# jluuser/PyTorch-VAE

Hardware: AMD Instinct MI355X
Metric: train images/sec @64x64x3 bs256 (curve tensors [B,64,6], SURVEY.md s0) (higher is better)
Workload: dtype f32; 1 GPU; C2: stage2_vq.yaml model with num_quantizers=1 K=512 D=64 N=64; full train step (fwd+loss+bwd+clip+AdamW+EMA), dropout 0.1, loss weights at epoch 100; per_gpu_batch=256, global_batch=256, seq_len=64, parallelism=dp1, hipgraph=True, params=43115078

## Files before the change

pytorch-vae_amd/csrc/gemm_dma.inc:

```

namespace dma {
constexpr int TBM = 256, TBN = 128, TBK = 32;
constexpr int A_BYTES = TBM * TBK * 4, B_BYTES = TBN * TBK * 4, STAGE_BYTES = A_BYTES + B_BYTES;
constexpr int NSTAGE = 3, LDS_BYTES = NSTAGE * STAGE_BYTES;
constexpr int DMA_A = A_BYTES / 1024 / 4, DMA_B = B_BYTES / 1024 / 4, DMA_PER_WAVE = DMA_A + DMA_B;
constexpr int MI = 4, NJ = 2;
}

typedef float f32x2 __attribute__((ext_vector_type(2)));

typedef unsigned u32x2 __attribute__((ext_vector_type(2)));
typedef unsigned u32x4 __attribute__((ext_vector_type(4)));
typedef short s16x4 __attribute__((ext_vector_type(4)));
typedef __bf16 bf16x8 __attribute__((ext_vector_type(8)));

namespace x3 {
constexpr int A_PLANE = dma::TBM * dma::TBK * 2, B_PLANE = dma::TBN * dma::TBK * 2;
constexpr int B_OFF = 3 * A_PLANE;
constexpr int STAGE_BYTES = 3 * (A_PLANE + B_PLANE);
constexpr int LDS_BYTES = 2 * STAGE_BYTES;
constexpr int NU = 12, NUA = 8;
constexpr int NB = 8, G = 48, NSLOT = 96;
constexpr int BAR = 7 * NU;
constexpr int RS_OFF = 40960;
static_assert(LDS_BYTES <= dma::LDS_BYTES, "x3 stages must fit the launch's dynamic LDS");
}

template <class F, int... I>
__device__ __forceinline__ void static_for_impl(F&& f, std::integer_sequence<int, I...>) { (f(std::integral_constant<int, I>{}), ...); }
template <int N, class F>
__device__ __forceinline__ void static_for(F&& f) { static_for_impl(f, std::make_integer_sequence<int, N>{}); }

struct SplitUnit {
    float r0, r1, r2, r3;
    unsigned t0, t1, t2, t3;
    unsigned hp[2], mp[2], lp[2];
    template <int S> __device__ __forceinline__ void step(const f32x4& a) {
        if constexpr (S == 0) {
            asm volatile("v_cvt_pk_bf16_f32 %0, %6, %7\n\tv_cvt_pk_bf16_f32 %1, %8, %9\n\tv_lshlrev_b32 %2, 16, %0\n\t"
                         "v_and_b32 %3, 0xffff0000, %0\n\tv_sub_f32 %4, %6, %2\n\tv_sub_f32 %5, %7, %3"
                         : "=&v"(hp[0]), "=&v"(hp[1]), "=&v"(t0), "=&v"(t1), "=&v"(r0), "=&v"(r1)
                         : "v"(a[0]), "v"(a[1]), "v"(a[2]), "v"(a[3]) : "memory");
        } else if constexpr (S == 1) {
            asm volatile("v_lshlrev_b32 %0, 16, %6\n\tv_and_b32 %1, 0xffff0000, %6\n\tv_sub_f32 %2, %7, %0\n\t"
                         "v_sub_f32 %3, %8, %1\n\tv_cvt_pk_bf16_f32 %4, %9, %10\n\tv_cvt_pk_bf16_f32 %5, %2, %3"
                         : "=&v"(t2), "=&v"(t3), "=&v"(r2), "=&v"(r3), "=&v"(mp[0]), "=&v"(mp[1])
                         : "v"(hp[1]), "v"(a[2]), "v"(a[3]), "v"(r0), "v"(r1) : "memory");
        } else if constexpr (S == 2) {
            asm volatile("v_lshlrev_b32 %0, 16, %2\n\tv_and_b32 %1, 0xffff0000, %2" : "=&v"(t0), "=&v"(t1) : "v"(mp[0]) : "memory");
        } else if constexpr (S == 3) {
            asm volatile("v_sub_f32 %0, %0, %2\n\tv_sub_f32 %1, %1, %3" : "+v"(r0), "+v"(r1) : "v"(t0), "v"(t1) : "memory");
        } else if constexpr (S == 4) {
            asm volatile("v_lshlrev_b32 %0, 16, %6\n\tv_and_b32 %1, 0xffff0000, %6\n\tv_sub_f32 %2, %2, %0\n\t"
                         "v_sub_f32 %3, %3, %1\n\tv_cvt_pk_bf16_f32 %4, %7, %8\n\tv_cvt_pk_bf16_f32 %5, %2, %3"
                         : "=&v"(t2), "=&v"(t3), "+v"(r2), "+v"(r3), "=&v"(lp[0]), "=&v"(lp[1])
                         : "v"(mp[1]), "v"(r0), "v"(r1) : "memory");
        }
    }
    __device__ __forceinline__ void all(const f32x4& a) { step<0>(a); step<1>(a); step<2>(a); step<3>(a); step<4>(a); }
};

__device__ __forceinline__ void glds16_s(const char* ubase, unsigned voff, unsigned lds_byte_addr_uniform) {
    asm volatile("s_mov_b32 m0, %2\n\ts_nop 0\n\tglobal_load_lds_dwordx4 %0, %1"
                 :
                 : "v"(voff), "s"(ubase), "s"(lds_byte_addr_uniform)
                 : "memory");
}

__device__ __forceinline__ void glds16(const float* gptr, unsigned lds_byte_addr_uniform) {
    __builtin_amdgcn_global_load_lds(gptr, (__attribute__((address_space(3))) void*)(uintptr_t)lds_byte_addr_uniform, 16, 0, 0);
}

template <bool A_KC, bool B_KC, int MODE, bool X3 = false>
__device__ __forceinline__ void gemm_dma_tile(const GemmArgs& g, const int tile, const int zsplit) {
    using namespace dma;
    constexpr bool EA_KC = X3 ? true : A_KC, EB_KC = X3 ? true : B_KC;
    extern __shared__ __attribute__((aligned(1024))) unsigned char smem_dma[];
    const int tid = threadIdx.x, lane = tid & 63;
    const int wave = __builtin_amdgcn_readfirstlane(tid >> 6);
    const int wm = wave >> 1, wn = wave & 1;
    const int l31 = lane & 31, h = lane >> 5;

    const int tiles_n = g.N / TBN;
    const int m0 = (tile / tiles_n) * TBM, n0 = (tile % tiles_n) * TBN;
    const int kbeg = zsplit * g.kchunk;
    const int kend = min(g.K, kbeg + g.kchunk);
    const int nk = (kend - kbeg) / TBK;

    unsigned voff[DMA_PER_WAVE];
    unsigned dst[DMA_PER_WAVE];
#pragma unroll
    for (int i = 0; i < DMA_A; ++i) {
        const int j = wave + 4 * i;
        if (A_KC) {
            const int R = j * 8 + (lane >> 3), c = (lane & 7) ^ ((R >> 1) & 7);
            voff[i] = (unsigned)(((size_t)R * g.lda + c * 4) * 4);
        } else {
            voff[i] = (unsigned)(((size_t)j * g.lda + lane * 4) * 4);
        }
        dst[i] = j * 1024;
    }
#pragma unroll
    for (int i = 0; i < DMA_B; ++i) {
        const int j = wave + 4 * i;
        if (B_KC) {
            const int R = j * 8 + (lane >> 3), c = (lane & 7) ^ ((R >> 1) & 7);
            voff[DMA_A + i] = (unsigned)(((size_t)R * g.ldb + c * 4) * 4);
        } else {
            voff[DMA_A + i] = (unsigned)(((size_t)(2 * j + (lane >> 5)) * g.ldb + (lane & 31) * 4) * 4);
        }
        dst[DMA_A + i] = A_BYTES + j * 1024;
    }
    const char* baseA = reinterpret_cast<const char*>(A_KC ? g.A + (size_t)m0 * g.lda + kbeg : g.A + (size_t)kbeg * g.lda + m0);
    const char* baseB = reinterpret_cast<const char*>(B_KC ? g.B + (size_t)n0 * g.ldb + kbeg : g.B + (size_t)kbeg * g.ldb + n0);
    const size_t stepA = (A_KC ? (size_t)TBK : (size_t)TBK * g.lda) * 4;
    const size_t stepB = (B_KC ? (size_t)TBK : (size_t)TBK * g.ldb) * 4;
    const unsigned lds0 = (unsigned)(uintptr_t)smem_dma;

    const int sw = (l31 >> 1) & 7;
    unsigned offA[4], offB[4];
#pragma unroll
    for (int t = 0; t < 4; ++t) {
        offA[t] = A_KC ? (unsigned)((wm * 128 + l31) * 128 + (((2 * t + h) ^ sw) * 16))
                       : (unsigned)((8 * t + 4 * h) * (TBM * 4) + (wm * 128 + 4 * l31) * 4);
        offB[t] = A_BYTES + (B_KC ? (unsigned)((wn * 64 + l31) * 128 + (((2 * t + h) ^ sw) * 16))
                                  : (unsigned)((8 * t + 4 * h) * (TBN * 4) + (wn * 64 + 2 * l31) * 4));
    }

    f32x16 acc[MI][NJ];
#pragma unroll
    for (int i = 0; i < MI; ++i)
#pragma unroll
        for (int j = 0; j < NJ; ++j)
#pragma unroll
            for (int r = 0; r < 16; ++r) acc[i][j][r] = 0.f;

    f32x4 fa[2][4];
    f32x4 fbk[2][2];
    f32x2 fbr[2][4];
    const bool do_rowsum = (!A_KC) && (g.rowsum != nullptr) && (n0 == 0) && (X3 || wn == 0);
    float rs[4] = {0.f, 0.f, 0.f, 0.f};

    constexpr int NREAD = 4 + (B_KC ? 2 : 4);
    constexpr int NMF = 4 * MI * NJ;
    constexpr int GAP = NMF / (NREAD + 1);
    auto substep = [&](auto c_c, auto rt_c, auto v0_c, auto v1_c, int rstage, int kt_d, int dstage) {
        constexpr int c = decltype(c_c)::value, RT = decltype(rt_c)::value, V0 = decltype(v0_c)::value,
                      V1 = decltype(v1_c)::value, n = c ^ 1;
        const unsigned char* sb = smem_dma + rstage * STAGE_BYTES;
        const unsigned dsb = lds0 + dstage * STAGE_BYTES;
        if (do_rowsum) {
#pragma unroll
            for (int e = 0; e < 4; ++e)
#pragma unroll
                for (int i = 0; i < 4; ++i) rs[i] += fa[c][e][i];
        }
#pragma unroll
        for (int m = 0; m < NMF; ++m) {
            const int e = m / (MI * NJ), i = (m / NJ) % MI, j = m % NJ;
            const float av = A_KC ? fa[c][i][e] : fa[c][e][i];
            const float bv = B_KC ? fbk[c][j][e] : fbr[c][e][j];
            acc[i][j] = __builtin_amdgcn_mfma_f32_32x32x2f32(av, bv, acc[i][j], 0, 0, 0);
            if ((m % GAP) == 0 && m / GAP < NREAD) {
                const int d = m / GAP;
                if (d < 4) {
                    fa[n][d] = *reinterpret_cast<const f32x4*>(sb + offA[RT] + (A_KC ? d * 32 * 128 : d * TBM * 4));
                } else if (B_KC) {
                    fbk[n][d - 4] = *reinterpret_cast<const f32x4*>(sb + offB[RT] + (d - 4) * 32 * 128);
                } else {
                    fbr[n][d - 4] = *reinterpret_cast<const f32x2*>(sb + offB[RT] + (d - 4) * TBN * 4);
                }
            }
            if ((m % GAP) == GAP / 2 && V0 + m / GAP < V1) {
                const int v = V0 + m / GAP;
                const char* ub = (v < DMA_A) ? baseA + (size_t)kt_d * stepA : baseB + (size_t)kt_d * stepB;
                glds16_s(ub, voff[v], __builtin_amdgcn_readfirstlane(dsb + dst[v]));
            }
        }
#pragma unroll
        for (int m = 0; m < NMF; ++m) {
            __builtin_amdgcn_sched_group_barrier(0x008, 1, 0);
            if ((m % GAP) == 0 && m / GAP < NREAD) __builtin_amdgcn_sched_group_barrier(0x100, 1, 0);
            if ((m % GAP) == GAP / 2 && V0 + m / GAP < V1) __builtin_amdgcn_sched_group_barrier(0x020, 1, 0);
        }
    };
    auto read_first = [&](int rstage) {
        const unsigned char* sb = smem_dma + rstage * STAGE_BYTES;
#pragma unroll
        for (int d = 0; d < 4; ++d) fa[0][d] = *reinterpret_cast<const f32x4*>(sb + offA[0] + (A_KC ? d * 32 * 128 : d * TBM * 4));
        if (B_KC) {
#pragma unroll
            for (int d = 0; d < 2; ++d) fbk[0][d] = *reinterpret_cast<const f32x4*>(sb + offB[0] + d * 32 * 128);
        } else {
#pragma unroll
            for (int d = 0; d < 4; ++d) fbr[0][d] = *reinterpret_cast<const f32x2*>(sb + offB[0] + d * TBN * 4);
        }
    };
    auto issue_all = [&](int kt, int stage) {
        const unsigned sbb = lds0 + stage * STAGE_BYTES;
#pragma unroll
        for (int v = 0; v < DMA_PER_WAVE; ++v) {
            const char* ub = (v < DMA_A) ? baseA + (size_t)kt * stepA : baseB + (size_t)kt * stepB;
            glds16_s(ub, voff[v], __builtin_amdgcn_readfirstlane(sbb + dst[v]));
        }
    };

    const int c4 = (lane & 15) * 4;
    const int col = n0 + wn * 64 + c4;
    constexpr bool HAS_DROP = (MODE == EPI_RELU_DROP || MODE == EPI_DROP_RESID);
    constexpr bool HAS_AUX = (MODE == EPI_DROP_RESID || MODE > EPI_SIGMOID);
    unsigned dkey = 0;
    if (g.drop.p > 0.f && g.drop.rng_state) dkey = drop_key(g.drop, g.drop.rng_state[0], g.drop.rng_state[1]);
    unsigned dmask[4] = {0u, 0u, 0u, 0u};
    const unsigned pair0 = (unsigned)((((unsigned long long)(m0 + wm * 128 + (lane >> 4)) * g.N + col) >> 2) * 2);
    const unsigned g0 = pair0 * 0x9E3779B9U;
    const unsigned gstep = (unsigned)(2 * g.N) * 0x9E3779B9U;
    auto hash_quad = [&](int qi) {
        const unsigned gq = g0 + (unsigned)qi * gstep;
        const unsigned b0 = mix32(dkey ^ gq), b1 = mix32(dkey ^ (gq + 0x9E3779B9U));
        unsigned f4 = ((b0 & 0xffffu) >= g.drop.thr) ? 1u : 0u;
        f4 |= ((b0 >> 16) >= g.drop.thr) ? 2u : 0u;
        f4 |= ((b1 & 0xffffu) >= g.drop.thr) ? 4u : 0u;
        f4 |= ((b1 >> 16) >= g.drop.thr) ? 8u : 0u;
        const unsigned sh = f4 << ((qi & 7) * 4);
        const int w = qi >> 3;
#pragma unroll
        for (int k = 0; k < 4; ++k) dmask[k] |= (w == k) ? sh : 0u;
    };
    f32x4 auxr[32];
    auto load_aux_all = [&]() {
        const float* ap = g.aux_in + (size_t)(m0 + wm * 128 + (lane >> 4)) * g.ldaux + col;
#pragma unroll
        for (int q = 0; q < 32; ++q) auxr[q] = *reinterpret_cast<const f32x4*>(ap + (size_t)(q * 4) * g.ldaux);
    };

    using I0 = std::integral_constant<int, 0>;
    using I1 = std::integral_constant<int, 1>;
    using I2 = std::integral_constant<int, 2>;
    using I3 = std::integral_constant<int, 3>;
    using IH = std::integral_constant<int, DMA_PER_WAVE / 2>;
    using IF = std::integral_constant<int, DMA_PER_WAVE>;
    if constexpr (X3) {
        const unsigned vA = A_KC ? (unsigned)(((size_t)(8 * wave + (lane >> 3)) * g.lda + 4 * (lane & 7)) * 4)
                                 : (unsigned)(((size_t)(8 * wave) * g.lda + 4 * lane) * 4);
        const unsigned vB = B_KC ? (unsigned)(((size_t)(8 * wave + (lane >> 3)) * g.ldb + 4 * (lane & 7)) * 4)
                                 : (unsigned)(((size_t)(8 * wave + (lane >> 5)) * g.ldb + 4 * (lane & 31)) * 4);
        const size_t uA = (A_KC ? (size_t)32 * g.lda : (size_t)g.lda) * 4;
        const size_t uB = (B_KC ? (size_t)32 * g.ldb : (size_t)2 * g.ldb) * 4;
        unsigned wA[4], wB[2];
        {
            const int R = 8 * wave + (lane >> 3), c = (lane & 7) >> 1;
            const unsigned wkc = (unsigned)(R * 64 + ((c ^ ((R >> 2) & 3)) * 16) + (lane & 1) * 8);
#pragma unroll
            for (int x = 0; x < 4; ++x) wA[x] = A_KC ? wkc : (unsigned)((8 * wave) * 512 + (((lane >> 3) ^ x) * 64) + (lane & 7) * 8);
#pragma unroll
            for (int x = 0; x < 2; ++x)
                wB[x] = B_KC ? wkc
                             : (unsigned)((8 * wave + (lane >> 5)) * 256 + ((((lane >> 3) & 3) ^ ((2 * x + (lane >> 5)) & 3)) * 64) + (lane & 7) * 8);
        }
        unsigned rA[4], rB[2];
        {
            const int q = (lane & 15) >> 2, p = lane & 3, sub = (lane >> 4) & 1;
            if (A_KC) {
                const int R = wm * 128 + l31, f = (l31 >> 2) & 3;
                rA[0] = (unsigned)(R * 64 + ((h ^ f) * 16));
                rA[1] = (unsigned)(R * 64 + (((2 + h) ^ f) * 16));
                rA[2] = rA[3] = 0;
            } else {
#pragma unroll
                for (int i = 0; i < 4; ++i) rA[i] = (unsigned)((8 * h + q) * 512 + (((wm * 4 + i) ^ q) * 64) + (16 * sub + 4 * p) * 2);
            }
            if (B_KC) {
                const int R = wn * 64 + l31, f = (l31 >> 2) & 3;
                rB[0] = (unsigned)(R * 64 + ((h ^ f) * 16));
                rB[1] = (unsigned)(R * 64 + (((2 + h) ^ f) * 16));
            } else {
#pragma unroll
                for (int j = 0; j < 2; ++j) rB[j] = (unsigned)((8 * h + q) * 256 + (((wn * 2 + j) ^ q) * 64) + (16 * sub + 4 * p) * 2);
            }
        }
        f32x4 st[x3::NU];
        u32x4 xA[3][4];
        u32x4 xB[2][3][2];
        SplitUnit su;
        auto load_unit = [&](auto u_c, int kt) {
            constexpr int u = decltype(u_c)::value;
            if constexpr (u < x3::NUA) st[u] = *reinterpret_cast<const f32x4*>(baseA + (size_t)kt * stepA + (size_t)u * uA + vA);
            else st[u] = *reinterpret_cast<const f32x4*>(baseB + (size_t)kt * stepB + (size_t)(u - x3::NUA) * uB + vB);
        };
        auto write_unit = [&](auto u_c, auto pl_c, unsigned char* sb) {
            constexpr int u = decltype(u_c)::value, pl = decltype(pl_c)::value;
            const u32x2 v = pl == 0 ? u32x2{su.hp[0], su.hp[1]} : pl == 1 ? u32x2{su.mp[0], su.mp[1]} : u32x2{su.lp[0], su.lp[1]};
            if constexpr (u < x3::NUA) {
                constexpr int cst = A_KC ? u * 2048 : u * 512;
                *reinterpret_cast<u32x2*>(sb + pl * x3::A_PLANE + cst + wA[A_KC ? 0 : (u & 3)]) = v;
            } else {
                constexpr int i = u - x3::NUA;
                constexpr int cst = B_KC ? i * 2048 : 2 * i * 256;
                *reinterpret_cast<u32x2*>(sb + x3::B_OFF + pl * x3::B_PLANE + cst + wB[B_KC ? 0 : (i & 1)]) = v;
            }
        };
        auto read_A = [&](auto pl_c, auto i_c, auto g_c, const unsigned char* sb) -> u32x4 {
            constexpr int pl = decltype(pl_c)::value, i = decltype(i_c)::value, gg = decltype(g_c)::value;
            if constexpr (A_KC) {
                return *reinterpret_cast<const u32x4*>(sb + pl * x3::A_PLANE + i * 2048 + rA[gg]);
            } else {
                const unsigned a0 = (unsigned)(uintptr_t)(sb + pl * x3::A_PLANE + (16 * gg) * 512 + rA[i]);
                const s16x4 lo = __builtin_amdgcn_ds_read_tr16_b64_v4i16((__attribute__((address_space(3))) s16x4*)(uintptr_t)a0);
                const s16x4 hi = __builtin_amdgcn_ds_read_tr16_b64_v4i16((__attribute__((address_space(3))) s16x4*)(uintptr_t)(a0 + 4 * 512));
                const u32x2 l2 = __builtin_bit_cast(u32x2, lo), h2 = __builtin_bit_cast(u32x2, hi);
                return u32x4{l2[0], l2[1], h2[0], h2[1]};
            }
        };
        auto read_B = [&](auto pl_c, auto j_c, auto g_c, const unsigned char* sb) -> u32x4 {
            constexpr int pl = decltype(pl_c)::value, j = decltype(j_c)::value, gg = decltype(g_c)::value;
            if constexpr (B_KC) {
                return *reinterpret_cast<const u32x4*>(sb + x3::B_OFF + pl * x3::B_PLANE + j * 2048 + rB[gg]);
            } else {
                const unsigned a0 = (unsigned)(uintptr_t)(sb + x3::B_OFF + pl * x3::B_PLANE + (16 * gg) * 256 + rB[j]);
                const s16x4 lo = __builtin_amdgcn_ds_read_tr16_b64_v4i16((__attribute__((address_space(3))) s16x4*)(uintptr_t)a0);
                const s16x4 hi = __builtin_amdgcn_ds_read_tr16_b64_v4i16((__attribute__((address_space(3))) s16x4*)(uintptr_t)(a0 + 4 * 256));
                const u32x2 l2 = __builtin_bit_cast(u32x2, lo), h2 = __builtin_bit_cast(u32x2, hi);
                return u32x4{l2[0], l2[1], h2[0], h2[1]};
            }
        };
        auto aux_one = [&](auto q_c) {
            constexpr int q = decltype(q_c)::value;
            auxr[q] = *reinterpret_cast<const f32x4*>(g.aux_in + (size_t)(m0 + wm * 128 + (lane >> 4) + q * 4) * g.ldaux + col);
        };
        if (nk > 0) {
            static_for<x3::NU>([&](auto u_c) { load_unit(u_c, 0); });
            if (HAS_DROP && g.drop.p > 0.f && !g.ws) {
#pragma unroll
                for (int qi = 0; qi < 32; ++qi) hash_quad(qi);
            }
            static_for<x3::NU>([&](auto u_c) {
                constexpr int u = decltype(u_c)::value;
                if (do_rowsum && u < x3::NUA) {
#pragma unroll
                    for (int e = 0; e < 4; ++e) rs[e] += st[u][e];
                }
                su.all(st[u]);
                write_unit(u_c, I0{}, smem_dma);
                write_unit(u_c, I1{}, smem_dma);
                write_unit(u_c, I2{}, smem_dma);
                load_unit(u_c, nk > 1 ? 1 : 0);
            });
            asm volatile("s_waitcnt lgkmcnt(0)" ::: "memory");
            __builtin_amdgcn_s_barrier();
            static_for<4>([&](auto i_c) { xA[0][decltype(i_c)::value] = read_A(I0{}, i_c, I0{}, smem_dma); });
            static_for<6>([&](auto x_c) {
                constexpr int x = decltype(x_c)::value;
                xB[0][x / 2][x % 2] = read_B(std::integral_constant<int, x / 2>{}, std::integral_constant<int, x % 2>{}, I0{}, smem_dma);
            });
            auto kstep = [&](auto last_c, const int kt) {
                constexpr bool LAST = decltype(last_c)::value;
                const unsigned char* rstg = smem_dma + (kt & 1) * x3::STAGE_BYTES;
                unsigned char* wstg = smem_dma + ((kt & 1) ^ 1) * x3::STAGE_BYTES;
                const int kt_ld = min(kt + 2, nk - 1);
                const bool want_aux = LAST && HAS_AUX && !g.ws;
                static_for<x3::NSLOT>([&](auto m_c) {
                    constexpr int m = decltype(m_c)::value;
                    constexpr int gg = m / x3::G, mm = m % x3::G, pi = mm / x3::NB, b = mm % x3::NB, i = b / 2, j = b % 2;
                    constexpr int pa = (pi < 3) ? 0 : (pi < 5) ? 1 : 2;
                    constexpr int pb = (pi == 0 || pi == 3 || pi == 5) ? 0 : (pi == 1 || pi == 4) ? 1 : 2;
                    acc[i][j] = __builtin_amdgcn_mfma_f32_32x32x16_bf16(__builtin_bit_cast(bf16x8, xA[pa][i]),
                                                                        __builtin_bit_cast(bf16x8, xB[gg][pb][j]), acc[i][j], 0, 0, 0);
                    if constexpr (m < 8 && m % 2 == 0) xA[1][m / 2] = read_A(I1{}, std::integral_constant<int, m / 2>{}, I0{}, rstg);
                    if constexpr (m >= 8 && m < 16 && m % 2 == 0) xA[2][(m - 8) / 2] = read_A(I2{}, std::integral_constant<int, (m - 8) / 2>{}, I0{}, rstg);
                    if constexpr (m >= 16 && m < 28 && m % 2 == 0) {
                        constexpr int x = (m - 16) / 2;
                        xB[1][x / 2][x % 2] = read_B(std::integral_constant<int, x / 2>{}, std::integral_constant<int, x % 2>{}, I1{}, rstg);
                    }
                    if constexpr (m >= 28 && m < 44 && m % 4 == 0) xA[0][(m - 28) / 4] = read_A(I0{}, std::integral_constant<int, (m - 28) / 4>{}, I1{}, rstg);
                    if constexpr (m >= 48 && m < 56 && m % 2 == 0) xA[1][(m - 48) / 2] = read_A(I1{}, std::integral_constant<int, (m - 48) / 2>{}, I1{}, rstg);
                    if constexpr (m >= 56 && m < 64 && m % 2 == 0) xA[2][(m - 56) / 2] = read_A(I2{}, std::integral_constant<int, (m - 56) / 2>{}, I1{}, rstg);
                    if constexpr (!LAST) {
                        if constexpr (m >= x3::BAR && m < x3::BAR + 4) xA[0][m - x3::BAR] = read_A(I0{}, std::integral_constant<int, m - x3::BAR>{}, I0{}, wstg);
                        if constexpr (m >= x3::BAR + 4 && m < x3::BAR + 10) {
                            constexpr int x = m - x3::BAR - 4;
                            xB[0][x / 2][x % 2] = read_B(std::integral_constant<int, x / 2>{}, std::integral_constant<int, x % 2>{}, I0{}, wstg);
                        }
                        if constexpr (m < x3::BAR) {
                            constexpr int u = m / 7, ph = m % 7;
                            using U = std::integral_constant<int, u>;
                            if constexpr (ph == 0) {
                                if (do_rowsum && u < x3::NUA) {
#pragma unroll
                                    for (int e = 0; e < 4; ++e) rs[e] += st[u][e];
                                }
                                su.template step<0>(st[u]);
                            }
                            if constexpr (ph == 1) su.template step<1>(st[u]);
                            if constexpr (ph == 2) { su.template step<2>(st[u]); write_unit(U{}, I0{}, wstg); }
                            if constexpr (ph == 3) { su.template step<3>(st[u]); write_unit(U{}, I1{}, wstg); }
                            if constexpr (ph == 4) load_unit(U{}, kt_ld);
                            if constexpr (ph == 5) su.template step<4>(st[u]);
                            if constexpr (ph == 6) write_unit(U{}, I2{}, wstg);
                        }
                        if constexpr (m == x3::BAR - 1) {
                            asm volatile("s_waitcnt lgkmcnt(0)" ::: "memory");
                            __builtin_amdgcn_s_barrier();
                        }
                    } else if constexpr (HAS_AUX) {
                        if constexpr (m % 3 == 0) {
                            if (want_aux) aux_one(std::integral_constant<int, m / 3>{});
                        }
                    }
                    __builtin_amdgcn_sched_barrier(0);
                });
            };
            for (int kt = 0; kt < nk - 1; ++kt) kstep(std::false_type{}, kt);
            kstep(std::true_type{}, nk - 1);
            __builtin_amdgcn_s_barrier();
        } else if (HAS_AUX && !g.ws) {
            load_aux_all();
        }
    } else
    if (nk > 0) {
        issue_all(0, 0);
        issue_all(nk > 1 ? 1 : 0, 1);
        if (HAS_DROP && g.drop.p > 0.f && !g.ws) {
#pragma unroll
            for (int qi = 0; qi < 32; ++qi) hash_quad(qi);
        }
        asm volatile("s_waitcnt vmcnt(%0)" ::"n"(DMA_PER_WAVE) : "memory");
        __builtin_amdgcn_s_barrier();
        read_first(0);
        int stage = 0;
        for (int kt = 0; kt < nk; ++kt) {
            const int nxt = (stage == 2) ? 0 : stage + 1;
            const int nx2 = (nxt == 2) ? 0 : nxt + 1;
            if (HAS_AUX && !g.ws && kt == nk - 1) load_aux_all();
            substep(I0{}, I1{}, I0{}, I0{}, stage, 0, 0);
            substep(I1{}, I2{}, I0{}, I0{}, stage, 0, 0);
            asm volatile("s_waitcnt vmcnt(0)" ::: "memory");
            __builtin_amdgcn_s_barrier();
            const int ktd = min(kt + 2, nk - 1);
            substep(I0{}, I3{}, I0{}, IH{}, stage, ktd, nx2);
            substep(I1{}, I0{}, IH{}, IF{}, nxt, ktd, nx2);
            stage = nxt;
        }
        asm volatile("s_waitcnt vmcnt(0)" ::: "memory");
        __builtin_amdgcn_s_barrier();
    } else if (HAS_AUX && !g.ws) {
        load_aux_all();
    }

    if (X3 && do_rowsum) {
        float* rsb = reinterpret_cast<float*>(smem_dma + x3::RS_OFF);
        *reinterpret_cast<f32x4*>(rsb + wave * TBM + 4 * lane) = f32x4{rs[0], rs[1], rs[2], rs[3]};
        __builtin_amdgcn_s_barrier();
        if (wave == 0) {
            f32x4 t = *reinterpret_cast<const f32x4*>(rsb + 4 * lane);
#pragma unroll
            for (int w = 1; w < 4; ++w) t += *reinterpret_cast<const f32x4*>(rsb + w * TBM + 4 * lane);
            const int row = m0 + 4 * lane;
            if (g.rowsum_ws) {
                *reinterpret_cast<f32x4*>(g.rowsum_ws + (size_t)zsplit * g.M + row) = t;
            } else {
#pragma unroll
                for (int i = 0; i < 4; ++i) g.rowsum[row + i] = (g.beta != 0.f) ? g.beta * g.rowsum[row + i] + t[i] : t[i];
            }
        }
    } else
    if (do_rowsum) {
#pragma unroll
        for (int i = 0; i < 4; ++i) rs[i] += __shfl_xor(rs[i], 32, 64);
        if (h == 0) {
            const int row = m0 + wm * 128 + 4 * l31;
            if (g.rowsum_ws) {
                *reinterpret_cast<f32x4*>(g.rowsum_ws + (size_t)zsplit * g.M + row) = f32x4{rs[0], rs[1], rs[2], rs[3]};
            } else {
#pragma unroll
                for (int i = 0; i < 4; ++i)
                    g.rowsum[row + i] = (g.beta != 0.f) ? g.beta * g.rowsum[row + i] + rs[i] : rs[i];
            }
        }
    }

    const int mode = (MODE >= 0) ? MODE : g.mode;
    constexpr int EP_LD = 68;
    float* ep = reinterpret_cast<float*>(smem_dma) + wave * (32 * EP_LD);
    float* slab = g.ws ? g.ws + (size_t)zsplit * g.M * g.N : nullptr;
    if constexpr (X3 && MODE == EPI_LINEAR) {
        if (!(g.flags & 2048)) {
            const size_t ldo = slab ? (size_t)g.N : (size_t)g.ldc;
            float* obase = slab ? slab : g.C;
#pragma unroll
            for (int j = 0; j < NJ; ++j) {
                const int cj = n0 + wn * 64 + j * 32 + l31;
                const float bj = (g.bias && !slab) ? g.bias[cj] : 0.f;
                float* cp = obase + (size_t)(m0 + wm * 128 + 4 * h) * ldo + cj;
                if (!slab && g.beta != 0.f) {
#pragma unroll
                    for (int i = 0; i < MI; ++i)
#pragma unroll
                        for (int r = 0; r < 16; ++r) {
                            float* q = cp + (size_t)(i * 32 + (r & 3) + 8 * (r >> 2)) * ldo;
                            *q = acc[i][j][r] + bj + g.beta * *q;
                        }
                } else {
#pragma unroll
                    for (int i = 0; i < MI; ++i)
#pragma unroll
                        for (int r = 0; r < 16; ++r) cp[(size_t)(i * 32 + (r & 3) + 8 * (r >> 2)) * ldo] = acc[i][j][r] + bj;
                }
            }
            return;
        }
    }
    f32x4 bias4 = {0.f, 0.f, 0.f, 0.f};
    if (mode <= EPI_SIGMOID && g.bias && !slab) bias4 = *reinterpret_cast<const f32x4*>(g.bias + col);
#pragma unroll
    for (int grp = 0; grp < 4; ++grp) {
        __builtin_amdgcn_wave_barrier();
#pragma unroll
        for (int q = 0; q < 16; ++q) {
            int rr, i, r;
            if (EA_KC) { i = grp; r = q; rr = (q & 3) + 8 * (q >> 2) + 4 * h; }
            else { i = q >> 2; r = 4 * grp + (q & 3); rr = 4 * ((q & 3) + 4 * h) + i; }
            if (EB_KC) {
                ep[rr * EP_LD + l31] = acc[i][0][r];
                ep[rr * EP_LD + 32 + l31] = acc[i][1][r];
            } else {
                *reinterpret_cast<f32x2*>(ep + rr * EP_LD + 2 * l31) = f32x2{acc[i][0][r], acc[i][1][r]};
            }
        }
        __builtin_amdgcn_s_waitcnt(0xC07F);
        __builtin_amdgcn_wave_barrier();
        constexpr int EPI_UNROLL = (MODE >= 0) ? 8 : 1;
#pragma unroll EPI_UNROLL
        for (int it = 0; it < 8; ++it) {
            const int rl = it * 4 + (lane >> 4);
            const int row = m0 + wm * 128 + grp * 32 + rl;
            f32x4 v = *reinterpret_cast<const f32x4*>(ep + rl * EP_LD + c4);
            if (slab) {
                *reinterpret_cast<f32x4*>(slab + (size_t)row * g.N + col) = v;
                continue;
            }
            float* cptr = g.C + (size_t)row * g.ldc + col;
            if (mode <= EPI_SIGMOID) {
                v += bias4;
                if (mode == EPI_RELU_DROP || mode == EPI_DROP_RESID) {
                    if (mode == EPI_RELU_DROP)
#pragma unroll
                        for (int e = 0; e < 4; ++e) v[e] = fmaxf(v[e], 0.f);
                    if (g.drop.p > 0.f) {
                        if (HAS_DROP) {
#pragma unroll
                            for (int e = 0; e < 4; ++e) v[e] = ((dmask[grp] >> (it * 4 + e)) & 1u) ? v[e] * g.drop.scale : 0.f;
                        } else {
                            float f[4];
                            drop4(g.drop, dkey, ((unsigned long long)row * g.N + col) >> 2, f);
#pragma unroll
                            for (int e = 0; e < 4; ++e) v[e] *= f[e];
                        }
                    }
                    if (mode == EPI_DROP_RESID)
                        v += HAS_AUX ? auxr[grp * 8 + it] : *reinterpret_cast<const f32x4*>(g.aux_in + (size_t)row * g.ldaux + col);
                } else if (mode == EPI_GELU) {
                    *reinterpret_cast<f32x4*>(g.aux_out + (size_t)row * g.ldaux + col) = v;
#pragma unroll
                    for (int e = 0; e < 4; ++e) v[e] = gelu_erf(v[e]);
                } else if (mode == EPI_SIGMOID) {
#pragma unroll
                    for (int e = 0; e < 4; ++e) v[e] = 1.f / (1.f + __expf(-v[e]));
                }
            } else {
                const f32x4 a = HAS_AUX ? auxr[grp * 8 + it] : *reinterpret_cast<const f32x4*>(g.aux_in + (size_t)row * g.ldaux + col);
                if (mode == EPI_MUL_POSMASK) {
#pragma unroll
                    for (int e = 0; e < 4; ++e) v[e] = (a[e] > 0.f) ? v[e] * g.drop.scale : 0.f;
                } else if (mode == EPI_MUL_GELUGRAD) {
#pragma unroll
                    for (int e = 0; e < 4; ++e) v[e] *= gelu_erf_grad(a[e]);
                } else {
#pragma unroll
                    for (int e = 0; e < 4; ++e) v[e] *= a[e] * (1.f - a[e]);
                }
            }
            if (g.beta != 0.f) v += g.beta * *reinterpret_cast<const f32x4*>(cptr);
            *reinterpret_cast<f32x4*>(cptr) = v;
        }
        __builtin_amdgcn_s_waitcnt(0xC07F);
    }
}

template <bool A_KC, bool B_KC, int MODE>
__global__ __launch_bounds__(256, 1) void gemm_f32_dma(const GemmArgs g) {
    const int nx = gridDim.x, nt = nx * gridDim.z, lin = blockIdx.z * nx + blockIdx.x;
    const int q = nt >> 3, r = nt & 7, x = lin & 7, j = lin >> 3;
    const int v = (x < r ? x * (q + 1) : r * (q + 1) + (x - r) * q) + j;
    gemm_dma_tile<A_KC, B_KC, MODE>(g, v % nx, v / nx);
}

template <bool A_KC, bool B_KC, int MODE>
__global__ __launch_bounds__(256, 1) void gemm_f32_x3(const GemmArgs g) {
    const int nx = gridDim.x, nt = nx * gridDim.z, lin = blockIdx.z * nx + blockIdx.x;
    const int q = nt >> 3, r = nt & 7, x = lin & 7, j = lin >> 3;
    const int v = (x < r ? x * (q + 1) : r * (q + 1) + (x - r) * q) + j;
    gemm_dma_tile<A_KC, B_KC, MODE, true>(g, v % nx, v / nx);
}

constexpr int GROUP_MAX = 8;
struct GemmGroupArgs {
    int n;
    int wg_begin[GROUP_MAX + 1];
    int tiles[GROUP_MAX];
    GemmArgs p[GROUP_MAX];
};

__device__ __forceinline__ int group_logical_id() {
    const int nt = gridDim.x, lin = blockIdx.x;
    const int q = nt >> 3, r = nt & 7, x = lin & 7, j = lin >> 3;
    return (x < r ? x * (q + 1) : r * (q + 1) + (x - r) * q) + j;
}

__global__ __launch_bounds__(256, 1) void gemm_f32_dma_group(const GemmGroupArgs G) {
    const int v = ((G.p[0].flags & 1) && !(G.p[0].flags & 1024)) ? group_logical_id() : (int)blockIdx.x;
    int p = 0;
    while (p + 1 < G.n && v >= G.wg_begin[p + 1]) ++p;
    const int local = v - G.wg_begin[p];
    const int tiles = G.tiles[p];
    gemm_dma_tile<false, false, EPI_LINEAR>(G.p[p], local % tiles, local / tiles);
}
__global__ __launch_bounds__(256, 1) void gemm_f32_x3_group(const GemmGroupArgs G) {
    const int v = ((G.p[0].flags & 1) && !(G.p[0].flags & 1024)) ? group_logical_id() : (int)blockIdx.x;
    int p = 0;
    while (p + 1 < G.n && v >= G.wg_begin[p + 1]) ++p;
    const int local = v - G.wg_begin[p];
    const int tiles = G.tiles[p];
    gemm_dma_tile<false, false, EPI_LINEAR, true>(G.p[p], local % tiles, local / tiles);
}
```

Measured before the change: 9762 images/s.

## Add register-direct epilogue for x3 GEMM tiles with aux prefetch in last k-step

Adds a specialised path for the x3 (split-bf16) GEMM kernel in which the epilogue for ReLU-dropout, GELU, dropout-residual and posmask modes writes accumulators straight from registers to global memory, skipping the shared-memory staging pass. Aux input values are prefetched into registers in the MFMA slots of the final k-step, and the dropout masks are redistributed through a small LDS exchange. The path is taken at runtime only when there is no split-K, no workspace, beta is zero and a flag bit is clear. In exchange the output stores are uncoalesced scalar writes, and holding 128 extra floats of aux in registers adds register pressure.

```diff
diff --git a/pytorch-vae_amd/csrc/gemm_dma.inc b/pytorch-vae_amd/csrc/gemm_dma.inc
--- a/pytorch-vae_amd/csrc/gemm_dma.inc
+++ b/pytorch-vae_amd/csrc/gemm_dma.inc
@@ -71,7 +71,11 @@
     __builtin_amdgcn_global_load_lds(gptr, (__attribute__((address_space(3))) void*)(uintptr_t)lds_byte_addr_uniform, 16, 0, 0);
 }
 
-template <bool A_KC, bool B_KC, int MODE, bool X3 = false>
+constexpr bool epi_has_direct(int mode) {
+    return mode == EPI_RELU_DROP || mode == EPI_GELU || mode == EPI_DROP_RESID || mode == EPI_MUL_POSMASK;
+}
+
+template <bool A_KC, bool B_KC, int MODE, bool X3 = false, bool DIR = false>
 __device__ __forceinline__ void gemm_dma_tile(const GemmArgs& g, const int tile, const int zsplit) {
     using namespace dma;
     constexpr bool EA_KC = X3 ? true : A_KC, EB_KC = X3 ? true : B_KC;
@@ -234,6 +238,81 @@
         for (int q = 0; q < 32; ++q) auxr[q] = *reinterpret_cast<const f32x4*>(ap + (size_t)(q * 4) * g.ldaux);
     };
 
+    static_assert(!DIR || (X3 && A_KC && epi_has_direct(MODE)), "register-direct epilogue: specialised x3 tiles only");
+    float auxd[128];
+    float bdir[NJ] = {0.f, 0.f};
+    auto drow = [](int i, int r) { return i * 32 + (r & 3) + 8 * (r >> 2); };
+    const char* auxbase = nullptr;
+    unsigned auxvoff = 0;
+    if (DIR && HAS_AUX) {
+        auxbase = reinterpret_cast<const char*>(g.aux_in + (size_t)(m0 + wm * 128) * g.ldaux + (n0 + wn * 64));
+        auxvoff = (unsigned)((4 * h * g.ldaux + l31) * 4);
+    }
+    auto aux_dir = [&](auto d_c) {
+        constexpr int d = decltype(d_c)::value, i = d / 32, r = (d / 2) % 16, j = d % 2;
+        const unsigned vo = auxvoff + (unsigned)(drow(i, r) * 4) * (unsigned)g.ldaux;
+        auxd[d] = *reinterpret_cast<const float*>(auxbase + (size_t)vo + j * 128);
+    };
+
+    auto direct_epilogue = [&]() {
+        u32x4 mw[NJ][4];
+        const bool dropping = HAS_DROP && __float_as_int(g.drop.p) > 0;
+        if (dropping) {
+            u32x4* mx = reinterpret_cast<u32x4*>(smem_dma) + wave * 64;
+            mx[lane] = u32x4{dmask[0], dmask[1], dmask[2], dmask[3]};
+            __builtin_amdgcn_s_waitcnt(0xC07F);
+            __builtin_amdgcn_wave_barrier();
+            const unsigned lsh = (unsigned)(4 * h + (l31 & 3));
+#pragma unroll
+            for (int j = 0; j < NJ; ++j)
+#pragma unroll
+                for (int rq = 0; rq < 4; ++rq) {
+                    const u32x4 w = mx[(rq << 4) | ((32 * j + l31) >> 2)];
+                    mw[j][rq] = u32x4{w[0] >> lsh, w[1] >> lsh, w[2] >> lsh, w[3] >> lsh};
+                }
+        }
+        char* const cbase = reinterpret_cast<char*>(g.C + (size_t)(m0 + wm * 128) * g.ldc + (n0 + wn * 64));
+        const unsigned cvoff = (unsigned)((4 * h * g.ldc + l31) * 4);
+        char* xbase = nullptr;
+        unsigned xvoff = 0;
+        if constexpr (MODE == EPI_GELU) {
+            xbase = reinterpret_cast<char*>(g.aux_out + (size_t)(m0 + wm * 128) * g.ldaux + (n0 + wn * 64));
+            xvoff = (unsigned)((4 * h * g.ldaux + l31) * 4);
+        }
+        const float scale = g.drop.scale;
+        auto store_all = [&](auto drop_c) {
+            constexpr bool DROP = decltype(drop_c)::value;
+#pragma unroll
+            for (int i = 0; i < MI; ++i)
+#pragma unroll
+                for (int r = 0; r < 16; ++r) {
+                    const unsigned co = cvoff + (unsigned)(drow(i, r) * 4) * (unsigned)g.ldc;
+                    const unsigned xo = xvoff + (unsigned)(drow(i, r) * 4) * (unsigned)g.ldaux;
+#pragma unroll
+                    for (int j = 0; j < NJ; ++j) {
+                        const int d = 32 * i + 2 * r + j;
+                        float v = acc[i][j][r];
+                        if constexpr (MODE <= EPI_SIGMOID) v = __fadd_rn(v, bdir[j]);
+                        if constexpr (MODE == EPI_RELU_DROP) v = fmaxf(v, 0.f);
+                        if constexpr (DROP) v = ((mw[j][r & 3][i] >> (8 * (r >> 2))) & 1u) ? __fmul_rn(v, scale) : 0.f;
+                        if constexpr (MODE == EPI_DROP_RESID) v = __fadd_rn(v, auxd[d]);
+                        if constexpr (MODE == EPI_GELU) {
+                            *reinterpret_cast<float*>(xbase + (size_t)xo + j * 128) = v;
+                            v = gelu_erf(v);
+                        }
+                        if constexpr (MODE == EPI_MUL_POSMASK) v = (auxd[d] > 0.f) ? __fmul_rn(v, scale) : 0.f;
+                        *reinterpret_cast<float*>(cbase + (size_t)co + j * 128) = v;
+                    }
+                }
+        };
+        if constexpr (HAS_DROP) {
+            if (dropping) store_all(std::true_type{});
+            else store_all(std::false_type{});
+        } else {
+            store_all(std::false_type{});
+        }
+    };
+
     using I0 = std::integral_constant<int, 0>;
     using I1 = std::integral_constant<int, 1>;
     using I2 = std::integral_constant<int, 2>;
@@ -353,8 +432,8 @@
                 constexpr int x = decltype(x_c)::value;
                 xB[0][x / 2][x % 2] = read_B(std::integral_constant<int, x / 2>{}, std::integral_constant<int, x % 2>{}, I0{}, smem_dma);
             });
-            auto kstep = [&](auto last_c, const int kt) {
-                constexpr bool LAST = decltype(last_c)::value;
+            auto kstep = [&](auto last_c, auto dir_c, const int kt) {
+                constexpr bool LAST = decltype(last_c)::value, AUXD = decltype(dir_c)::value;
                 const unsigned char* rstg = smem_dma + (kt & 1) * x3::STAGE_BYTES;
                 unsigned char* wstg = smem_dma + ((kt & 1) ^ 1) * x3::STAGE_BYTES;
                 const int kt_ld = min(kt + 2, nk - 1);
@@ -402,6 +481,13 @@
                             asm volatile("s_waitcnt lgkmcnt(0)" ::: "memory");
                             __builtin_amdgcn_s_barrier();
                         }
+                    } else if constexpr (HAS_AUX && AUXD) {
+                        if constexpr (m < 64) {
+                            aux_dir(m_c);
+                        } else {
+                            aux_dir(std::integral_constant<int, 2 * m - 64>{});
+                            aux_dir(std::integral_constant<int, 2 * m - 63>{});
+                        }
                     } else if constexpr (HAS_AUX) {
                         if constexpr (m % 3 == 0) {
                             if (want_aux) aux_one(std::integral_constant<int, m / 3>{});
@@ -410,8 +496,20 @@
                     __builtin_amdgcn_sched_barrier(0);
                 });
             };
-            for (int kt = 0; kt < nk - 1; ++kt) kstep(std::false_type{}, kt);
-            kstep(std::true_type{}, nk - 1);
+            for (int kt = 0; kt < nk - 1; ++kt) kstep(std::false_type{}, std::false_type{}, kt);
+            if constexpr (DIR) {
+                if constexpr (MODE <= EPI_SIGMOID) {
+                    if (g.bias) {
+#pragma unroll
+                        for (int j = 0; j < NJ; ++j) bdir[j] = g.bias[n0 + wn * 64 + j * 32 + l31];
+                    }
+                }
+                kstep(std::true_type{}, std::bool_constant<HAS_AUX>{}, nk - 1);
+                __builtin_amdgcn_s_barrier();
+                direct_epilogue();
+                return;
+            }
+            kstep(std::true_type{}, std::false_type{}, nk - 1);
             __builtin_amdgcn_s_barrier();
         } else if (HAS_AUX && !g.ws) {
             load_aux_all();
@@ -600,6 +698,14 @@
     const int nx = gridDim.x, nt = nx * gridDim.z, lin = blockIdx.z * nx + blockIdx.x;
     const int q = nt >> 3, r = nt & 7, x = lin & 7, j = lin >> 3;
     const int v = (x < r ? x * (q + 1) : r * (q + 1) + (x - r) * q) + j;
+    if constexpr (A_KC && epi_has_direct(MODE)) {
+        const bool direct = !(g.flags & 2048) && (__float_as_uint(g.beta) << 1) == 0u && !g.ws && gridDim.z == 1 &&
+                            g.K >= dma::TBK && g.kchunk >= dma::TBK && g.ldc < (1 << 22) && g.ldaux < (1 << 22);
+        if (direct) {
+            gemm_dma_tile<A_KC, B_KC, MODE, true, true>(g, v % nx, v / nx);
+            return;
+        }
+    }
     gemm_dma_tile<A_KC, B_KC, MODE, true>(g, v % nx, v / nx);
 }
 
```

New measurement: 9856 images/s (median of 6 runs). About the same (+1.0%).
